# baggepinnen/LPVSpectral.jl

Measured on AMD Instinct MI355X. Metric: signals/sec, ls_sparse_spectral_lpv group lasso N=2^20 Nf=512 Nv=8 (2000 ADMM iters; iters/sec in admm_iters_per_sec), higher is better.
Workload: dtype f64

## Files before the change

lpvspectral.jl_amd/csrc/admm.hip:

```cpp
#include "lpvs_internal.h"
#include "admm_device.h"
#include "admm_host.h"

#include <algorithm>
#include <map>
#include <mutex>
#include <tuple>
#include <vector>
#include <cmath>
#include <cstdlib>
#include <string>
#include <type_traits>

namespace lpvs {

namespace {

template <int RPW>
__global__ void __launch_bounds__(256)
symv_kernel(const double *__restrict__ M, int64_t np, const double *__restrict__ rhs_all, double *__restrict__ x_all,
            const AdmmStatus *status) {
    const int sg = blockIdx.y;
    if (status != nullptr && status[sg].converged) return;
    const double *rhs = rhs_all + (int64_t)sg * np;
// ... 1536 lines not shown
void launch_symv_raw(const double *M, int64_t np, const double *rhs, double *x, const AdmmStatus *st, int ns,
                            hipStream_t s) {
    if (np >= 4096)
        hipLaunchKernelGGL(symv_kernel<4>, dim3((unsigned)ceil_div(np, 16), (unsigned)ns), dim3(256), 0, s, M, np, rhs, x, st);
    else
        hipLaunchKernelGGL(symv_kernel<1>, dim3((unsigned)ceil_div(np, 4), (unsigned)ns), dim3(256), 0, s, M, np, rhs, x, st);
}

int32_t launch_symv(const double *M, int64_t np, const double *rhs, double *x, hipStream_t s, int ns) {
    launch_symv_raw(M, np, rhs, x, nullptr, ns, s);
    LPVS_HIP(hipGetLastError());
    return LPVS_OK;
}
__global__ void __launch_bounds__(256)
rhs_from_state_kernel(const double *__restrict__ z, const double *__restrict__ u, double mu, int64_t n, int64_t np, double *__restrict__ rhs) {
    const int64_t i = (int64_t)blockIdx.x * 256 + threadIdx.x;
    if (i < np) rhs[i] = i < n ? (z[i] - u[i]) / mu : 0.0;
}
__global__ void __launch_bounds__(256)
vec_diff_kernel(const double *a, const double *b, double *out, int64_t total) {
    const int64_t i = (int64_t)blockIdx.x * 256 + threadIdx.x;
    if (i < total) out[i] = a[i] - b[i];
}
int32_t launch_nibble_refresh(const AdmmParams &p, bool from_state, const double *u_src, hipStream_t s, bool split) {
    if (p.ns != 1 || p.mp_types == nullptr || p.xb_corr == nullptr || p.nib_rhs == nullptr || p.nib_part == nullptr) { set_error("nibble refresh: not a single-signal mixed-storage handle"); return LPVS_ESTATE; }
    const int nblk = (int)(p.np / TS);
    const unsigned ntiles = (unsigned)(nblk * (nblk + 1) / 2);
    double *part1 = p.nib_part, *part2 = part1 + (size_t)ntiles * TS;
    const double *rhs = p.rhs;
    if (from_state) {
        hipLaunchKernelGGL(rhs_from_state_kernel, dim3((unsigned)ceil_div(p.np, 256)), dim3(256), 0, s, p.z, u_src, p.mu, p.n, p.np, p.nib_rhs);
        rhs = p.nib_rhs;
    }
    launch_split(reinterpret_cast<const unsigned char *>(p.Mp), p.mp_types, rhs, p.np, ntiles, part1, part2, nullptr, s, 2);
    if (split) {
        hipLaunchKernelGGL(symv_reduce_kernel, dim3((unsigned)nblk, 1u), dim3(256), 0, s, part1, part2, nblk, (int)ntiles, p.np, p.nib_rhs, nullptr, (const double *)nullptr, 0);
        hipLaunchKernelGGL(vec_diff_kernel, dim3((unsigned)ceil_div(p.np, 256)), dim3(256), 0, s, p.xb, (const double *)p.nib_rhs, const_cast<double *>(p.xb_corr), p.np);
    } else
        hipLaunchKernelGGL(symv_reduce_kernel, dim3((unsigned)nblk, 1u), dim3(256), 0, s, part1, part2, nblk, (int)ntiles, p.np, const_cast<double *>(p.xb), nullptr, p.xb_corr, 0);
    LPVS_HIP(hipGetLastError());
    return LPVS_OK;
}

void launch_gather_tile_partials(const double *part1, const double *part2, int nblk, unsigned ntiles, int64_t np, double *out, hipStream_t s) {
    hipLaunchKernelGGL(symv_reduce_kernel, dim3((unsigned)nblk, 1u), dim3(256), 0, s, part1, part2, nblk, (int)ntiles, np, out, (const AdmmStatus *)nullptr, (const double *)nullptr, 0);
}
// ... 58 lines not shown
```

lpvspectral.jl_amd/csrc/admm_one_launch.hip:

```cpp
#include "lpvs_internal.h"
#include "admm_device.h"
#include "admm_host.h"

#include <algorithm>
#include <map>
#include <mutex>
#include <tuple>
#include <vector>
#include <cmath>
#include <cstdlib>
#include <string>
#include <type_traits>

namespace lpvs {

enum { FI_FIRST = 0, FI_MID = 1, FI_LAST = 2 };
typedef void (*FiKernel)(AdmmParams, const unsigned char *, const unsigned char *, int, int, long long, int, int, int, size_t, int);
static FiKernel fi_kernel(int mode, bool small, bool batch, bool nt, bool pa, bool f32);

__device__ __forceinline__ double wave_max(double v) {
#pragma unroll
    for (int o = 32; o > 0; o >>= 1) v = fmax(v, __shfl_xor(v, o, 64));
    return v;
}
// ... 180 lines not shown
        bnv[k] = MODE != FI_FIRST ? f.bn[pg * nbt + boff + b] : 0.0;
        recv[k] = MODE != FI_LAST ? f.rec[pg * nbt + boff + b] : make_double2(0.0, 0.0);
    }
    const double Rrow = BATCH ? f.consts[2 * sg] : p.fi_R, xbmax = BATCH ? f.consts[2 * sg + 1] : p.fi_xbmax;
    __builtin_amdgcn_sched_barrier(0);
    FixRaw fr;
    float4 fha[8], fhb[8];
    double diag_pre = 0.0;
    if (MODE != FI_LAST && F32) {
        typedef unsigned int u32x4b __attribute__((ext_vector_type(4)));
        const __amdgpu_buffer_rsrc_t rs = __builtin_amdgcn_make_buffer_rsrc(const_cast<unsigned char *>(tile), 0, TS * TS * 4, 0x00020000);
        const int off_head = ((wave * 32 + (lane >> 4)) * TS + 4 * (lane & 15)) * 4;
#pragma unroll
        for (int rg = 0; rg < 8; ++rg) {
            fha[rg] = __builtin_bit_cast(float4, (u32x4b)__builtin_amdgcn_raw_buffer_load_b128(rs, off_head, rg * (4 * TS * 4), 0));
            fhb[rg] = __builtin_bit_cast(float4, (u32x4b)__builtin_amdgcn_raw_buffer_load_b128(rs, off_head, rg * (4 * TS * 4) + 256, 0));
        }
    }
    if (MODE != FI_LAST && !F32) {
        typedef unsigned int u32x4b __attribute__((ext_vector_type(4)));
        constexpr int aux = NT ? 2 : 0;
        const int tbytes = I != J ? (int)kMixedFixedTileBytes : (prefetch_all ? (int)kMixedFixedTileBytes + TS * 8 : 0);
        const __amdgpu_buffer_rsrc_t rs = __builtin_amdgcn_make_buffer_rsrc(const_cast<unsigned char *>(tile), 0, tbytes, 0x00020000);
        const __amdgpu_buffer_rsrc_t rs_nq = __builtin_amdgcn_make_buffer_rsrc(const_cast<unsigned char *>(tile), 0, p.mp_fix32 ? 0 : tbytes, 0x00020000);
        const int gq_ = lane >> 4, c_ = lane & 15;
        const int off_head = ((wave * 32 + gq_) * TS + 4 * c_) * 4;
        const int off_nq = (int)kFixHeadBytes + (wave * 64 + lane) * 32, off_st = (int)(kFixHeadBytes + kFixNibBytes) + (wave * 4 + gq_) * 32;
        fr.nq[0] = __builtin_bit_cast(uint4, (u32x4b)__builtin_amdgcn_raw_buffer_load_b128(rs_nq, off_nq, 0, aux));
        fr.nq[1] = __builtin_bit_cast(uint4, (u32x4b)__builtin_amdgcn_raw_buffer_load_b128(rs_nq, off_nq, 16, aux));
        fr.st[0] = __builtin_bit_cast(float4, (u32x4b)__builtin_amdgcn_raw_buffer_load_b128(rs, off_st, 0, aux));
        fr.st[1] = __builtin_bit_cast(float4, (u32x4b)__builtin_amdgcn_raw_buffer_load_b128(rs, off_st, 16, aux));
#pragma unroll
        for (int rg = 0; rg < 8; ++rg) {
            fr.ha[rg] = __builtin_bit_cast(int4, (u32x4b)__builtin_amdgcn_raw_buffer_load_b128(rs, off_head, rg * (4 * TS * 4), aux));
            fr.hb[rg] = __builtin_bit_cast(int4, (u32x4b)__builtin_amdgcn_raw_buffer_load_b128(rs, off_head, rg * (4 * TS * 4) + 256, aux));
        }
        if (PA) {
            const int rgo = ((c_ & 8) ? 4 : 0) + ((c_ & 4) ? 2 : 0) + ((c_ & 2) ? 1 : 0);
            typedef unsigned int u32x2b __attribute__((ext_vector_type(2)));
            const u32x2b dw = __builtin_amdgcn_raw_buffer_load_b64(rs, (int)(kFixHeadBytes + kFixNibBytes) + TS * 4 + (wave * 32 + 4 * rgo + gq_) * 8, 0, 0);
            diag_pre = __builtin_bit_cast(double, dw);
        }
    }
    __builtin_amdgcn_sched_barrier(0);
    double mR = 0, mU = 0;
#pragma unroll
    for (int k = 0; k < NK; ++k) { mR = fmax(mR, recv[k].x); mU = fmax(mU, recv[k].y); }
// ... 53 lines not shown
            if (threadIdx.x == 0) {
                f.bn[pg1 * nbt + boff + I] = red[0][0] + red[0][1];
                f.rec[pg1 * nbt + boff + I] = make_double2(fmax(red[1][0], red[1][1]), fmax(red[2][0], red[2][1]));
            }
        }
    }
    if (MODE == FI_LAST) return;
    LPVS_TL_STAMP(2);
    if (I == J && threadIdx.x < TS) f.acc((aslot + 1) % 3)[voff + e] = 0;
    if (threadIdx.x < TS) sI[i] = rhs_v; else sJ[i] = rhs_v;
    mR = wave_max_nonneg(mR); mU = wave_max_nonneg(mU);
    double B = Rrow * ((xbmax + Rrow * mR + mU) / p.mu) * 1.000001;
    const bool bound_ok = B < 0x1p1000;
    if (!(B > 0x1p-900)) B = 0x1p-900;
    int eb = 0;
    (void)frexp(bound_ok ? B : 1.0, &eb);
    const double quantum = bound_ok ? ldexp(1.0, eb - 62) : __longlong_as_double(0x7ff8000000000000ll), invq = bound_ok ? ldexp(1.0, 62 - eb) : 0.0;
    if (blockIdx.x == 0 && threadIdx.x == 0) f.qbuf[pg * nprob + sg] = quantum;
    __syncthreads();
    LPVS_TL_STAMP(3);
    const int c = lane & 15, gq = lane >> 4;
    double rj[8], tc[8], v[8];
    const double *diag = nullptr;
    if (F32) {
#pragma unroll
        for (int k = 0; k < 4; ++k) { rj[k] = sJ[4 * c + k]; rj[4 + k] = sJ[64 + 4 * c + k]; }
#pragma unroll
        for (int k = 0; k < 8; ++k) tc[k] = 0.0;
#pragma unroll
        for (int rg = 0; rg < 8; ++rg) {
            const double ri = sI[wave * 32 + 4 * rg + gq];
            const float hh[8] = {fha[rg].x, fha[rg].y, fha[rg].z, fha[rg].w, fhb[rg].x, fhb[rg].y, fhb[rg].z, fhb[rg].w};
            double a0 = 0.0, a1 = 0.0;
#pragma unroll
            for (int k = 0; k < 8; k += 2) {
                const double m0 = (double)hh[k], m1 = (double)hh[k + 1];
                tc[k] = opaque(fma(m0, ri, tc[k]));
                tc[k + 1] = opaque(fma(m1, ri, tc[k + 1]));
                a0 = fma(m0, rj[k], a0);
                a1 = fma(m1, rj[k + 1], a1);
            }
            v[rg] = a0 + a1;
            __builtin_amdgcn_sched_barrier(0);
        }
    } else if (PA || ttype != 0) {
        if (!PA && I == J) {
            FixRaw fd;
            fix_load(tile, wave, lane, fd, p.mp_fix32 != 0 ? 1 : 0);
            fi_fixed_product(fd, sI, sJ, wave, lane, v, tc);
        } else fi_fixed_product(fr, sI, sJ, wave, lane, v, tc);
        if (ttype == 2 && !prefetch_all) diag = reinterpret_cast<const double *>(tile + kFixHeadBytes + kFixNibBytes + TS * 4);
    } else {
#pragma unroll
        for (int k = 0; k < 4; ++k) { rj[k] = sJ[4 * c + k]; rj[4 + k] = sJ[64 + 4 * c + k]; }
#pragma unroll
        for (int k = 0; k < 8; ++k) tc[k] = 0.0;
        const float *head = reinterpret_cast<const float *>(tile) + (wave * 32 + gq) * TS + 4 * c;
        const unsigned short *tail = reinterpret_cast<const unsigned short *>(tile + (size_t)TS * TS * 4) + (wave * 32 + gq) * TS + 8 * c;
#pragma unroll
        for (int half = 0; half < 2; ++half) {
            float4 ha[4], hb[4];
            uint4 lq[4];
#pragma unroll
            for (int r4 = 0; r4 < 4; ++r4) {
                const int rg = 4 * half + r4;
                ha[r4] = load16<NT, float4>(head + rg * 4 * TS);
                hb[r4] = load16<NT, float4>(head + rg * 4 * TS + 64);
                lq[r4] = load16<NT, uint4>(tail + rg * 4 * TS);
            }
// ... 37 lines not shown
    }
    if (I != J) {
#pragma unroll
        for (int m = 32, cnt = 4; m >= 16; m >>= 1, cnt >>= 1) {
            const bool up = (lane & m) != 0;
#pragma unroll
            for (int k = 0; k < cnt; ++k) {
                const double lo_ = opaque(tc[k]), hi_ = opaque(tc[k + cnt]);
                tc[k] = (up ? hi_ : lo_) + __shfl_xor(up ? lo_ : hi_, m, 64);
            }
        }
        const int col = ((lane & 32) ? 64 : 0) + 4 * c + ((lane & 16) ? 2 : 0);
        sT[wave][col] = tc[0]; sT[wave][col + 1] = tc[1];
        __syncthreads();
        if (threadIdx.x < TS) {
            const double r2 = ((sT[0][threadIdx.x] + sT[1][threadIdx.x]) + sT[2][threadIdx.x]) + sT[3][threadIdx.x];
            atomicAdd(acc_cur + voff + (int64_t)J * TS + threadIdx.x, (unsigned long long)__double2ll_rn(r2 * invq));
        }
    }
    if constexpr (NIBR && !F32) {
        if (ttype != 0) {
            __syncthreads();
            FixRaw fb;
            fix_load(tile, wave, lane, fb, 2);
            double vn[8], tn[8];
            fi_fixed_product(fb, sI, sJ, wave, lane, vn, tn);
            unsigned long long *acc_n = reinterpret_cast<unsigned long long *>(p.nib_acc);
#pragma unroll
            for (int m = 8, cnt = 4; m >= 2; m >>= 1, cnt >>= 1) {
                const bool up = (c & m) != 0;
#pragma unroll
                for (int k = 0; k < cnt; ++k) {
                    const double lo_ = opaque(vn[k]), hi_ = opaque(vn[k + cnt]);
                    vn[k] = (up ? hi_ : lo_) + __shfl_xor(up ? lo_ : hi_, m, 64);
                }
            }
            vn[0] += __shfl_xor(vn[0], 1, 64);
            if ((c & 1) == 0) {
                const int rg = ((c & 8) ? 4 : 0) + ((c & 4) ? 2 : 0) + ((c & 2) ? 1 : 0);
                atomicAdd(acc_n + voff + (int64_t)I * TS + wave * 32 + 4 * rg + gq, (unsigned long long)__double2ll_rn(vn[0] * invq));
            }
            if (I != J) {
#pragma unroll
                for (int m = 32, cnt = 4; m >= 16; m >>= 1, cnt >>= 1) {
                    const bool up = (lane & m) != 0;
#pragma unroll
                    for (int k = 0; k < cnt; ++k) {
// ... 150 lines not shown
```

lpvspectral.jl_amd/csrc/api.hip:

```cpp
#include <cmath>
#include <cstdarg>
#include <cstdio>
#include <cstdlib>
#include <cstring>
#include <ctime>
#include <map>
#include <mutex>
#include <array>
#include <thread>
#include <string>
#include <vector>

#include "lpvs_internal.h"

namespace lpvs {

static thread_local char g_err[512] = "";

void set_error(const char *fmt, ...) {
    va_list ap;
    va_start(ap, fmt);
    vsnprintf(g_err, sizeof(g_err), fmt, ap);
    va_end(ap);
}
// ... 425 lines not shown
                 h->rhs.as<double>(), h->mu, h->tol, h->prox_kind, h->prox_param, h->group_len, h->status.as<AdmmStatus>(),
                 h->scratch.as<double>(), h->part.as<double>(), sym ? h->Mp.as<double>() : nullptr, (int)h->ns};
    p.mp_f32 = sym && h->Mp_mode == kMpF32 ? 1 : 0;
    p.mp_split = sym && (h->Mp_mode == kMpSplit || h->Mp_mode == kMpMixed) ? 1 : 0;
    p.mp_types = sym && h->Mp_mode == kMpMixed ? h->Mp.as<unsigned char>() + 6 * symv_packed_doubles(h->np) : nullptr;
    p.mp_fix32 = p.mp_types != nullptr && (h->Mp_fix_bits <= 32 || h->nib_period > 0) ? 1 : 0;
    p.nib_period = p.mp_types != nullptr ? h->nib_period : 0; p.nib_ramp = h->nib_ramp; p.xb_corr = h->xb_corr.as<double>(); p.nib_rhs = h->nib_rhs.as<double>(); p.nib_part = h->nib_part.as<double>(); p.nib_acc = h->nib_acc.as<long long>();
    p.xb = sym && h->offset_form ? h->xb.as<double>() : nullptr;
    p.fi = sym && h->offset_form && h->ns == 1 && (h->Mp_mode == kMpMixed || h->Mp_mode == kMpF32) && h->fi.p ? h->fi.as<double>() : nullptr;
    p.fi_R = h->fi_R; p.fi_xbmax = h->fi_xbmax;
    p.fi_prefetch_all = sym && h->Mp_mode == kMpMixed && h->Mp_fixed_tiles == (int64_t)(symv_packed_doubles(h->np) / (128 * 128)) ? 1 : 0;
    p.opt_iteration = h->opt[LPVS_OPT_ITERATION]; p.opt_nt_loads = h->opt[LPVS_OPT_NT_LOADS];
    p.sm_ctl = !sym && h->sm_ctl.p ? h->sm_ctl.as<int>() : nullptr;
    return p;
}

int32_t factorize(lpvs_problem *h, double shift) {
    if (h->M_valid && h->M_shift == shift) return LPVS_OK;
    const int64_t np = h->np, n = h->n;
    h->Mp_valid = false; h->Mp_rowsum = 0;
    if (!h->M.p) LPVS_TRY(h->M.alloc(sizeof(double) * (size_t)np * (size_t)np));
    if (!h->work.p) LPVS_TRY(h->work.alloc(spd_inverse_work_bytes(np)));
    LPVS_HIP(hipEventRecord(h->ev[3].a, h->stream));
    LPVS_HIP(hipMemcpyAsync(h->M.p, h->G.p, sizeof(double) * (size_t)np * (size_t)np, hipMemcpyDeviceToDevice, h->stream));
    LPVS_TRY(launch_add_diag(h->M.as<double>(), np, n, shift, h->stream));
    LPVS_TRY(spd_inverse_inplace(h->M.as<double>(), np, h->work.as<double>(), h->istat.as<int>(), h->stream, &h->res->aux));
    LPVS_HIP(hipEventRecord(h->ev[3].b, h->stream));
    int st = 0;
    LPVS_HIP(hipMemcpyAsync(&st, h->istat.p, sizeof(int), hipMemcpyDeviceToHost, h->stream));
    LPVS_HIP(hipStreamSynchronize(h->stream));
    h->t_factor += h->ev[3].ms();
    if (st != 0) {
        h->M_valid = false;
        set_error("(G + %.3g I) is not positive definite (non-positive pivot in the block sweep)", shift);
        return LPVS_ENUMERIC;
    }
    h->M_valid = true; h->M_shift = shift;
    return LPVS_OK;
}

}

template <class Fill>
static int32_t create_panel_problem(lpvs_problem *h, const double *y, const double *W, int64_t N, Fill fill) {
    hipStream_t s = h->stream;
    h->np = round_up(h->n, 128);
    const GramPlan pl = make_gram_plan(h->n, N);
    const int64_t Npad = pl.ksplit * pl.rows_per_chunk;
// ... 235 lines not shown
        LPVS_TRY(copy_to_device(hi.p, sl.om_hi.data(), sizeof(double) * (size_t)sl.nsl, s));
        LPVS_TRY(copy_to_device(lo.p, sl.om_lo.data(), sizeof(double) * (size_t)sl.nsl, s));
        LPVS_TRY(copy_to_device(rhi.p, sl.omr_hi.data(), sizeof(double) * (size_t)sl.nf8, s));
        LPVS_TRY(copy_to_device(rlo.p, sl.omr_lo.data(), sizeof(double) * (size_t)sl.nf8, s));
        LPVS_TRY(copy_to_device(eps.p, sl.eps.data(), sizeof(double) * sl.eps.size(), s));
        return LPVS_OK;
    }
};

static int32_t create_lpv_impl(const double *y, int64_t ns, const double *X, const double *V, int64_t N, const double *w, int64_t Nf,
                               int64_t Nv, int32_t normalize, int32_t coulomb, int32_t device, lpvs_problem **out,
                               const double *ranges = nullptr) {
    if (N <= 0 || Nf <= 0 || Nv <= 0 || ns <= 0) { set_error("N, Nf, Nv and the number of signals must be positive"); return LPVS_EARGUMENT; }
    lpvs_problem *h = nullptr;
    LPVS_TRY(problem_begin(device, out, &h));
    struct Guard { lpvs_problem *h; ~Guard() { delete h; } } guard{h};
    hipStream_t s = h->stream;
    const int64_t nb = coulomb ? 2 * Nv : Nv;
    h->kind = 1; h->N = N; h->Nf = Nf; h->nb = nb; h->n = 2 * Nf * nb; h->np = round_up(h->n, 128); h->ns = ns;
    DevArg dy, dX, dV, dw;
    LPVS_TRY(dy.set(y, N * ns, s)); LPVS_TRY(dX.set(X, N, s)); LPVS_TRY(dV.set(V, N, s)); LPVS_TRY(dw.set(w, Nf, s));
    LPVS_TRY(h->G.alloc(sizeof(double) * (size_t)h->np * (size_t)h->np));
    LPVS_TRY(h->b.alloc(sizeof(double) * (size_t)h->np * (size_t)ns));
    LPVS_HIP(hipMemsetAsync(h->G.p, 0, h->G.bytes, s));
    LPVS_HIP(hipMemsetAsync(h->b.p, 0, h->b.bytes, s));
    LPVS_TRY(alloc_state(h));

    const int form_opt = option_in_effect(LPVS_OPT_GRAM_FORM, h->opt[LPVS_OPT_GRAM_FORM]);
    const std::string form = form_opt == LPVS_GRAM_AP ? "ap" : form_opt == LPVS_GRAM_KRS ? "krs" : form_opt == LPVS_GRAM_KR ? "kr" : "auto";
    bool use_ap = false;
    ApSlots sl;
    double xam = 0;
    if (form == "auto" || form == "ap") {
        std::vector<double> hw;
        LPVS_TRY(fetch_host(hw, w, Nf));
        double xlo, xhi;
        if (ranges) xam = ranges[3];
        else LPVS_TRY(device_minmax(dX.p, N, &xlo, &xhi, &xam, s));
        sl = make_ap_slots(hw, xam);
        use_ap = sl.ok;
        if (form == "ap" && !use_ap) { set_error("LPVS_GRAM_FORM=ap but w is not an arithmetic progression (max|eps|*max|x| = %.3g)", sl.emax * xam); return LPVS_EARGUMENT; }
    }
    if (use_ap) {
        const int64_t nf8 = sl.nf8, nsl = sl.nsl, P = nb * (nb + 1) / 2;
        const ApStep &step = sl.step;
        double lo, hi, am, gamma; std::vector<double> vc;
        DevBuf K, KK, dvc, part, tab, tabb, nwork, epsr;
        ApSlotsDev sd;
        DrainOnExit drain(s);
        LPVS_HIP(hipEventRecord(h->ev[0].a, s));
        if (ranges) { lo = ranges[0]; hi = ranges[1]; am = ranges[2]; }
        else LPVS_TRY(device_minmax(dV.p, N, &lo, &hi, &am, s));
        basis_centers(lo, hi, am, Nv, coulomb, vc, &gamma);
        const int64_t ldk = nb + 1;
        LPVS_TRY(dvc.alloc(sizeof(double) * vc.size()));
        LPVS_TRY(copy_to_device(dvc.p, vc.data(), sizeof(double) * vc.size(), s));
        LPVS_TRY(K.alloc(sizeof(double) * (size_t)N * (size_t)ldk));
        LPVS_TRY(KK.alloc(sizeof(double) * (size_t)N * (size_t)P));
        LPVS_TRY(launch_basis_table(dV.p, N, dvc.as<double>(), nb, gamma, normalize, coulomb, K.as<double>(), ldk, s));
        LPVS_TRY(launch_pair_table(K.as<double>(), ldk, nb, N, KK.as<double>(), s));
        LPVS_TRY(sd.upload(sl, s));
        LPVS_HIP(hipEventRecord(h->ev[0].b, s));
        LPVS_TRY(part.alloc(std::max(nudft_partial_bytes(N, nsl, P), nudft_partial_bytes(N, nf8, nb))));
        LPVS_TRY(tab.alloc(sizeof(double) * (size_t)nsl * (size_t)P * 4));
        LPVS_TRY(tabb.alloc(sizeof(double) * (size_t)nf8 * (size_t)nb * 4));
        LPVS_HIP(hipEventRecord(h->ev[1].a, s));
        const bool nufft_on = option_in_effect(LPVS_OPT_SLOT_SUMS, h->opt[LPVS_OPT_SLOT_SUMS]) != LPVS_SLOTS_DIRECT;
        bool nufft = nufft_on && sl.merged && nufft_applicable(N, nsl, P);
        const int nfg = nufft_grid_size(nsl);
        const double xam_ = xam;
        if (nufft) {
            LPVS_TRY(nwork.alloc(nufft_work_bytes(N, nsl, P)));
// ... 27 lines not shown
                if (rc == kNufftNonFinite) by_nufft = false;
                else if (rc != LPVS_OK) return rc;
            }
            if (!by_nufft)
                LPVS_TRY(launch_nudft(dX.p, dy.p + q * N, N, K.as<double>(), ldk, (int)nb, sd.rhi.as<double>(), sd.rlo.as<double>(), (int)nf8, step, part.as<double>(), tabb.as<double>(), s));
            LPVS_TRY(launch_ap_rhs(tabb.as<double>(), by_nufft ? epsr.as<double>() : sd.eps.as<double>(), Nf, nb, h->b.as<double>() + q * h->np, s));
        }
        LPVS_HIP(hipEventRecord(h->ev[2].b, s));
        LPVS_HIP(hipStreamSynchronize(s));
        h->t_basis = h->ev[0].ms(); h->t_gram = h->ev[1].ms(); h->t_reduce = h->ev[2].ms();
        h->gram_launches = 8.0 * (double)N * (double)nsl * (double)P;
        h->gram_flops = (double)N * (double)h->n * (double)(h->n + 1);
        guard.h = nullptr;
        *out = h;
        return LPVS_OK;
    }

    const bool krs = form != "kr" && gram_krs_fits(nb);
    const GramPlan pl = krs ? make_gram_plan_pairs(Nf, nb, N) : make_gram_plan(h->n, N);
    const int64_t Npad = pl.ksplit * pl.rows_per_chunk;

    DevBuf T, K, KK, G3, slab, scr; int64_t ldk;
    DrainOnExit drain(s);
    LPVS_HIP(hipEventRecord(h->ev[0].a, s));
    LPVS_TRY(build_lpv_tables(dX.p, dV.p, N, Npad, dw.p, Nf, Nv, normalize, coulomb, T, K, &ldk, s, ranges));
    if (krs) {
        LPVS_TRY(KK.alloc(sizeof(double) * (size_t)Npad * (size_t)pl.pairs));
        LPVS_TRY(launch_pair_table(K.as<double>(), ldk, nb, Npad, KK.as<double>(), s));
    }
    LPVS_HIP(hipEventRecord(h->ev[0].b, s));
    LPVS_TRY(slab.alloc(pl.slab_bytes));
    LPVS_TRY(scr.alloc(rhs_scratch_bytes(N, h->n)));
    if (krs) LPVS_TRY(G3.alloc(sizeof(double) * (size_t)pl.np2 * (size_t)(pl.np2 * pl.pairs)));
    struct Side { hipStream_t s = nullptr; hipEvent_t ready = nullptr, done = nullptr;
                  ~Side() { if (s) { (void)hipStreamSynchronize(s); (void)hipStreamDestroy(s); } if (ready) (void)hipEventDestroy(ready); if (done) (void)hipEventDestroy(done); } } side;
    LPVS_HIP(hipStreamCreateWithFlags(&side.s, hipStreamNonBlocking));
    LPVS_HIP(hipEventCreateWithFlags(&side.ready, hipEventDisableTiming));
    LPVS_HIP(hipEventCreateWithFlags(&side.done, hipEventDisableTiming));
    LPVS_HIP(hipEventRecord(side.ready, s));
    LPVS_HIP(hipStreamWaitEvent(side.s, side.ready, 0));
    LPVS_HIP(hipEventRecord(h->ev[1].a, s));
    if (krs) LPVS_TRY(launch_gram_krs(pl, T.as<double2>(), Nf, KK.as<double>(), nb, slab.as<double>(), s));
    else LPVS_TRY(launch_gram_kr(pl, T.as<double2>(), Nf, K.as<double>(), ldk, nb, slab.as<double>(), s));
    LPVS_HIP(hipEventRecord(h->ev[1].b, s));
    for (int64_t q = 0; q < ns; ++q)
        LPVS_TRY(launch_rhs_kr(T.as<double2>(), Nf, K.as<double>(), ldk, nb, dy.p + q * N, N, h->b.as<double>() + q * h->np, scr.as<double>(), scr.bytes, side.s));
// ... 303 lines not shown
            LPVS_HIP(hipStreamSynchronize(s));
            if (want_R) memcpy(&h->Mp_rowsum, &rbits, sizeof(double));
            size_t ndiag = 0;
            for (unsigned char t : ht) { h->Mp_fixed_tiles += t != 0; ndiag += t == 2; }
            h->Mp_fixed_diag = (int64_t)ndiag;
            h->Mp_stream_bytes = (double)h->Mp_fixed_tiles * (double)kMixedFixedTileBytes + (double)ndiag * 1024.0 +
                                 (double)(ntiles - (size_t)h->Mp_fixed_tiles) * (double)kMixedFloatTileBytes;
            const size_t nblk_ = (size_t)(h->np / 128);
            if (getenv("LPVS_TRACE")) fprintf(stderr, "[lpvs] mixed packing: %lld of %zu tiles fixed point (%zu diagonal), ns = %lld\n", (long long)h->Mp_fixed_tiles, ntiles, nblk_, (long long)h->ns);
            if (2 * (size_t)h->Mp_fixed_tiles < ntiles) {
                LPVS_TRY(launch_pack_tiles_split(h->M.as<double>(), h->np, h->Mp.as<unsigned char>(), s));
                h->Mp_fixed_tiles = 0; h->Mp_fixed_diag = 0;
                h->Mp_stream_bytes = 6.0 * (double)symv_packed_doubles(h->np);
                h->Mp_valid = true; h->Mp_mode = kMpSplit; h->Mp_demoted = true; just_demoted = true;
            }
        } else LPVS_TRY(launch_pack_tiles(h->M.as<double>(), h->np, h->Mp.as<double>(), s));
        if (!just_demoted) { h->Mp_valid = true; h->Mp_mode = mode; }
    }
    LPVS_HIP(hipMemsetAsync(h->part.p, 0, h->part.bytes, s));
    h->mu = mu; h->tol = tol; h->sign = linear_sign;
    const size_t v = sizeof(double) * (size_t)h->np * (size_t)h->ns;
    LPVS_HIP(hipMemsetAsync(h->x.p, 0, v, s));
    if (x0) LPVS_TRY(copy_state_in(h, h->x.p, x0));
    std::vector<double> hb((size_t)h->np * (size_t)h->ns, 0.0);
    LPVS_HIP(hipMemcpyAsync(hb.data(), h->b.p, v, hipMemcpyDeviceToHost, s));
    LPVS_HIP(hipStreamSynchronize(s));
    if (linear_sign < 0) for (auto &q : hb) q = -q;
    LPVS_TRY(copy_to_device(h->bs.p, hb.data(), v, s));
    h->offset_form = h->np >= kSymmetricMinNp;
    if (h->offset_form) {
        if (!h->xb.p) LPVS_TRY(h->xb.alloc(v));
        int steps = 1;
        if (const char *e = experiment_env("LPVS_XB_REFINE")) steps = atoi(e) < 0 ? 0 : atoi(e);
        h->xb_refined = steps > 0;
        LPVS_TRY(launch_offset_vector_refined(h->G.as<double>(), h->M.as<double>(), h->np, h->n, (int)h->ns, h->bs.as<double>(), h->M_shift, steps,
                                              h->xb.as<double>(), h->rhs.as<double>(), h->scratch.as<double>(), s));
        if (h->xcorr()) {
            if (!h->xb0.p) LPVS_TRY(h->xb0.alloc(v));
            if (!h->corr.p) LPVS_TRY(h->corr.alloc(3 * v));
            LPVS_HIP(hipMemcpyAsync(h->xb0.p, h->xb.p, v, hipMemcpyDeviceToDevice, s));
        }
        if (h->nib_period > 0 && h->Mp_mode == kMpMixed) {
            if (!h->xb_corr.p) LPVS_TRY(h->xb_corr.alloc(v));
            if (!h->nib_rhs.p) LPVS_TRY(h->nib_rhs.alloc(v));
            if (!h->nib_acc.p) LPVS_TRY(h->nib_acc.alloc(v));
            LPVS_HIP(hipMemsetAsync(h->nib_acc.p, 0, v, s));
            { const size_t nb = (size_t)(h->np / 128), nt = nb * (nb + 1) / 2; if (!h->nib_part.p) LPVS_TRY(h->nib_part.alloc(sizeof(double) * 2 * nt * 128)); }
            LPVS_HIP(hipMemcpyAsync(h->xb_corr.p, h->xb.p, v, hipMemcpyDeviceToDevice, s));
        } else h->nib_period = 0;
    } else { h->xcorr_base = 0; h->xcorr_every = 0; }
    h->k_enq = 0;
    if (h->offset_form && h->ns == 1 && (h->Mp_mode == kMpMixed || h->Mp_mode == kMpF32) && !h->fi.p) LPVS_TRY(h->fi.alloc(sizeof(double) * fi_doubles(h->np)));
    const AdmmParams p = make_params(h);
    LPVS_TRY(launch_admm_init(p, s));
    h->fi_sync = -1;
    if (p.fi) {
        if (h->Mp_rowsum > 0 && h->Mp_mode == kMpMixed) {
            AdmmParams pr = p; pr.fi_R = h->Mp_rowsum;
            LPVS_TRY(launch_fi_setup(pr, 0, true, s, h->Mp_rowsum));
        } else LPVS_TRY(launch_fi_setup(p, 0, true, s));
        double hc[2] = {0, 0};
        LPVS_TRY(fi_read_consts(p, hc, s));
        h->fi_R = hc[0]; h->fi_xbmax = hc[1] * (1.0 + 0x1p-20); h->fi_sync = 0;
    }
    LPVS_HIP(hipStreamSynchronize(s));
    h->inited = true;
    return LPVS_OK;
}

int32_t lpvs_admm_set_state_f64(lpvs_problem *h, const double *x, const double *z, const double *u, int64_t iters_done) {
    if (!h || !x || !z || !u) { set_error("NULL argument"); return LPVS_EARGUMENT; }
    if (!h->inited) { set_error("lpvs_admm_set_state before lpvs_admm_init"); return LPVS_ESTATE; }
    if (iters_done < 0) { set_error("iters_done must be >= 0"); return LPVS_EARGUMENT; }
    LPVS_HIP(hipSetDevice(h->device));
    hipStream_t s = h->stream;
    LPVS_TRY(copy_state_in(h, h->x.p, x));
    LPVS_TRY(copy_state_in(h, h->z.p, z));
    LPVS_TRY(copy_state_in(h, h->u.p, u));
    const AdmmParams p = make_params(h);
    LPVS_TRY(launch_admm_restate(p, iters_done, s));
    h->fi_sync = -1;
    h->k_enq = iters_done;
    if (h->xcorr() && iters_done == 0) {
        const size_t v = sizeof(double) * (size_t)h->np * (size_t)h->ns;
        LPVS_HIP(hipMemcpyAsync(h->xb.p, h->xb0.p, v, hipMemcpyDeviceToDevice, s));
        if (h->nib_period > 0 && h->xb_corr.p) {
            LPVS_HIP(hipMemcpyAsync(h->xb_corr.p, h->xb0.p, v, hipMemcpyDeviceToDevice, s));
            LPVS_HIP(hipMemsetAsync(h->nib_acc.p, 0, v, s));
// ... 1176 lines not shown
```

lpvspectral.jl_amd/csrc/linalg.hip:

```cpp
#include "lpvs_internal.h"

#include <cstdlib>
#include <map>
#include <mutex>
#include <string>
#include <vector>

namespace lpvs {

namespace {

typedef double f64x4 __attribute__((ext_vector_type(4)));
constexpr int NB = 64;

__global__ void __launch_bounds__(256)
diag_inverse_kernel(const double *__restrict__ Aall, int64_t np, int k, double *__restrict__ Pall, int *status,
                    int64_t strideA, int64_t strideW) {
    __shared__ double colp[NB], rowp[NB];
    const double *A = Aall + (int64_t)blockIdx.x * strideA;
    double *P = Pall + (int64_t)blockIdx.x * strideW;
    const double *blk = A + (int64_t)k * NB * np + (int64_t)k * NB;
    const int ti = threadIdx.x >> 4, tj = threadIdx.x & 15;
    double v[4][4];
#pragma unroll
// ... 871 lines not shown
#pragma unroll
            for (int r = 0; r < 4; ++r) {
                double *sp = A + (r_lo + i * 16 + 4 * r) * np + c_lo;
#pragma unroll
                for (int j = 0; j < 2; ++j) *reinterpret_cast<double *>(reinterpret_cast<char *>(sp + j * 16) + voffb) = acc[i][j][r];
            }
        return;
    }
#pragma unroll
    for (int i = 0; i < 2; ++i)
#pragma unroll
        for (int j = 0; j < 2; ++j)
#pragma unroll
            for (int r = 0; r < 4; ++r) {
                const int64_t row = r_lo + i * 16 + lk + 4 * r, col = c_lo + j * 16 + li;
                if (col <= row) A[row * np + col] = acc[i][j][r];
            }
}

__global__ void __launch_bounds__(256) add_diag_kernel(double *__restrict__ Mall, int64_t np, int64_t n, double shift) {
    const int64_t i = (int64_t)blockIdx.x * 256 + threadIdx.x;
    double *M = Mall + (int64_t)blockIdx.y * np * np;
    if (i < np) M[i * np + i] = i < n ? M[i * np + i] + shift : 1.0;
}

__global__ void __launch_bounds__(256) negate_mirror_kernel(double *__restrict__ Aall, int64_t np) {
    __shared__ double tile[32][33];
    double *A = Aall + (int64_t)blockIdx.z * np * np;
    const int bi = blockIdx.y, bj = blockIdx.x;
    if (bj > bi) return;
    const int tx = threadIdx.x & 31, ty = threadIdx.x >> 5;
    const int64_t r0 = (int64_t)bi * 32, c0 = (int64_t)bj * 32;
    for (int r = ty; r < 32; r += 8) {
        const double v = -A[(r0 + r) * np + c0 + tx];
        tile[r][tx] = v;
        if (bi != bj || tx <= r) A[(r0 + r) * np + c0 + tx] = v;
    }
    __syncthreads();
    for (int r = ty; r < 32; r += 8)
        if (bi != bj || tx > r) A[(c0 + r) * np + r0 + tx] = tile[tx][r];
}

__global__ void __launch_bounds__(256)
symm_matmul_kernel(const double *__restrict__ A, const double *__restrict__ B, double *__restrict__ C, int64_t np) {
    const int lane = threadIdx.x & 63, wave = threadIdx.x >> 6;
    const int64_t r0 = ((int64_t)blockIdx.y * 2 + (wave >> 1)) * 64, c0 = ((int64_t)blockIdx.x * 2 + (wave & 1)) * 64;
// ... 298 lines not shown
    } else {
        sweep64(A, np, nbatch, work, status_dev, s);
        LPVS_HIP(hipGetLastError());
    }
    hipLaunchKernelGGL(negate_mirror_kernel, dim3((unsigned)(np / 32), (unsigned)(np / 32), (unsigned)nbatch), dim3(256), 0, s, A, np);
    LPVS_HIP(hipGetLastError());
    return LPVS_OK;
}

int32_t spd_inverse_inplace_batch(double *A, int64_t np, int nbatch, double *work, int *status_dev, hipStream_t s) {
    return spd_inverse_impl(A, np, nbatch, work, status_dev, s, nullptr);
}

int32_t spd_inverse_inplace(double *A, int64_t np, double *work, int *status_dev, hipStream_t s, SweepAux *aux) {
    return spd_inverse_impl(A, np, 1, work, status_dev, s, aux);
}

int32_t launch_add_diag_batch(double *M, int64_t np, int64_t n, double shift, int nbatch, hipStream_t s) {
    hipLaunchKernelGGL(add_diag_kernel, dim3((unsigned)ceil_div(np, 256), (unsigned)nbatch), dim3(256), 0, s, M, np, n, shift);
    LPVS_HIP(hipGetLastError());
    return LPVS_OK;
}

int32_t launch_add_diag(double *M, int64_t np, int64_t n, double shift, hipStream_t s) {
    hipLaunchKernelGGL(add_diag_kernel, dim3((unsigned)ceil_div(np, 256)), dim3(256), 0, s, M, np, n, shift);
    LPVS_HIP(hipGetLastError());
    return LPVS_OK;
}

int32_t launch_symm_matmul(const double *A, const double *B, double *C, int64_t np, hipStream_t s) {
    if (np % 128 != 0) return LPVS_ESTATE;
    hipLaunchKernelGGL(symm_matmul_kernel, dim3((unsigned)(np / 128), (unsigned)(np / 128)), dim3(256), 0, s, A, B, C, np);
    LPVS_HIP(hipGetLastError());
    return LPVS_OK;
}

}
```

lpvspectral.jl_amd/csrc/lpvs_internal.h:

```cpp
#pragma once
#include <hip/hip_runtime.h>
#include <exception>
#include <new>
#include <stdint.h>
#include <functional>
#include <string>
#include <vector>

#include "../../include/lpvspectral.h"

namespace lpvs {

inline const char *experiment_env(const char *name) {
#ifdef LPVS_NO_EXPERIMENTS
    (void)name;
    return nullptr;
#else
    const char *on = getenv("LPVS_EXPERIMENTS");
    return (on && on[0] == '1') ? getenv(name) : nullptr;
#endif
}

void set_error(const char *fmt, ...);
#define LPVS_HIP(call)                                                                       \
// ... 125 lines not shown
std::vector<double> nufft_window_scale(int nf, int mode0, int nslots);
int32_t launch_nufft_window_spread(const double *x, const double *W, const double *yA, const double *yB, bool hasB, const int64_t *offs_dev, int nwin,
                                   int64_t n, double D_hi, double D_lo, int nf, double *gridA, double *gridB, int64_t grid_bstride, hipStream_t s);
int32_t launch_nufft_window_modes(const double *grids, int64_t grid_bstride, int nwin, int nf, int mode0, int nslots, const double *scale_dev, double *tab,
                                  int64_t tab_bstride, hipStream_t s);
int32_t launch_ap_assemble_fourier(const double *tab, const double *eps, int64_t Nf, int64_t s0, double delta, int zf, int64_t n, double *G,
                                   int64_t ldg, int nbatch, int64_t tab_stride, int64_t g_stride, hipStream_t s);
int32_t launch_ap_rhs_fourier(const double *tab, const double *eps, int64_t Nf, int zf, double *b, int nbatch, int64_t tab_stride,
                              int64_t b_stride, hipStream_t s);
int32_t launch_ap_assemble(const double *tab, const double *eps, int64_t Nf, int64_t s0, double delta, int64_t nb, int64_t n, double *G,
                           int64_t ldg, hipStream_t s);
int32_t launch_ap_rhs(const double *tab, const double *eps, int64_t Nf, int64_t nb, double *b, hipStream_t s);

struct SweepAux {
    hipStream_t side = nullptr;
    hipStream_t bulk = nullptr;
    hipEvent_t panel = nullptr, rest = nullptr, band = nullptr, second = nullptr, bulkdone = nullptr;
    int32_t ensure();
    ~SweepAux();
};
size_t spd_inverse_work_bytes(int64_t np);
int32_t spd_inverse_inplace(double *A, int64_t np, double *work, int *status_dev, hipStream_t s, SweepAux *aux = nullptr);
int32_t launch_add_diag(double *M, int64_t np, int64_t n, double shift, hipStream_t s);
int32_t launch_add_diag_batch(double *M, int64_t np, int64_t n, double shift, int nbatch, hipStream_t s);
int32_t spd_inverse_inplace_batch(double *A, int64_t np, int nbatch, double *work, int *status_dev, hipStream_t s);
int32_t launch_symm_matmul(const double *A, const double *B, double *C, int64_t np, hipStream_t s);

struct AdmmStatus {
    long long iters;
    int converged;
    int pad;
    double nxz;
};
struct AdmmParams {
    const double *M;
    int64_t np;
    int64_t n;
    const double *b;
    double *x, *z, *u, *rhs;
    double mu, tol;
    int prox_kind;
    double prox_param;
    int64_t group_len;
    AdmmStatus *status;
    double *scratch;
    double *part;
    const double *Mp;
    int ns;
    int mp_f32 = 0;
    int mp_split = 0;
    int nib_period = 0;
    int nib_ramp = 0;
    const double *xb_corr = nullptr;
    double *nib_rhs = nullptr;
    long long *nib_acc = nullptr;
    double *nib_part = nullptr;
    int mp_fix32 = 0;
    const unsigned char *mp_types = nullptr;
    const double *xb = nullptr;
    double *fi = nullptr;
    long long fi_base = 0;
    double fi_R = 0, fi_xbmax = 0;
    int fi_prefetch_all = 0;
    int opt_iteration = 0, opt_nt_loads = 0;
    int *sm_ctl = nullptr;
};
bool small_iter_applicable(const AdmmParams &p);
int32_t launch_nibble_refresh(const AdmmParams &p, bool from_state, const double *u_src, hipStream_t s, bool split = false);
inline bool nib_refresh_due(long long g, int period, int ramp) {
    if (period <= 0) return false;
    if (ramp <= 0) return g == 1 || g % period == 0;
    long long p2 = 1;
    while (2 * p2 <= g) p2 *= 2;
    long long step = p2 / ramp;
    if (step < 1) step = 1;
    if (step > period) step = period;
    return g % step == 0;
}
bool nib_fused_applies(const AdmmParams &p);
int32_t launch_xupdate_correction(const AdmmParams &p, const double *G, double shift, const double *b, const double *xb0, double *xb_eff, double *t, hipStream_t s);
size_t fi_doubles(int64_t np, int64_t nprob = 1);
bool fi_applicable(const AdmmParams &p);
int32_t launch_fi_setup(const AdmmParams &p, long long base, bool with_consts, hipStream_t s, double r_known = -1.0);
int32_t fi_read_consts(const AdmmParams &p, double out[2], hipStream_t s);
size_t symv_part_doubles(int64_t np, int64_t ns = 1);
size_t symv_packed_doubles(int64_t np);
int32_t launch_pack_tiles(const double *M, int64_t np, double *Mp, hipStream_t s);
int32_t launch_pack_tiles_f32(const double *M, int64_t np, float *Mp, hipStream_t s);
int32_t launch_pack_tiles_split(const double *M, int64_t np, unsigned char *Mp, hipStream_t s);
int32_t launch_pack_tiles_mixed(const double *M, int64_t np, unsigned char *Mp, unsigned char *types, unsigned long long *absmax, hipStream_t s,
                                bool diag_float = false, double *abs_part = nullptr, int64_t n_valid = 0, double *rows_scratch = nullptr, int fix_bits = 36);
// ... 81 lines not shown
```

Baseline: 14.33.

## Trim setup copies, memsets and host round-trips; reuse nibble tile loads

Setup now copies G into M in one fused kernel that adds the diagonal shift and touches only the lower-triangle tiles, replacing a full device-to-device copy plus a separate diagonal kernel. The sign flip of b runs on the device instead of going through a host round-trip. The full G memset becomes a memset of only the padding rows and columns on the Fourier path, and a redundant stream sync is dropped. In the fused iteration kernel, the nibble-refresh path reuses nibble and scale registers loaded earlier instead of reloading the tile. The lower-only copy assumes nothing reads M's upper triangle before the inverse, and it requires np to be a multiple of 128.

```diff
diff --git a/lpvspectral.jl_amd/csrc/admm.hip b/lpvspectral.jl_amd/csrc/admm.hip
--- a/lpvspectral.jl_amd/csrc/admm.hip
+++ b/lpvspectral.jl_amd/csrc/admm.hip
@@ -1582,6 +1582,16 @@
     const int64_t i = (int64_t)blockIdx.x * 256 + threadIdx.x;
     if (i < total) out[i] = a[i] - b[i];
 }
+__global__ void __launch_bounds__(256)
+signed_copy_kernel(const double *__restrict__ in, int negate, double *__restrict__ out, int64_t total) {
+    const int64_t i = (int64_t)blockIdx.x * 256 + threadIdx.x;
+    if (i < total) out[i] = negate ? -in[i] : in[i];
+}
+int32_t launch_signed_copy(const double *in, int sign, double *out, int64_t total, hipStream_t s) {
+    hipLaunchKernelGGL(signed_copy_kernel, dim3((unsigned)ceil_div(total, 256)), dim3(256), 0, s, in, sign < 0 ? 1 : 0, out, total);
+    LPVS_HIP(hipGetLastError());
+    return LPVS_OK;
+}
 int32_t launch_nibble_refresh(const AdmmParams &p, bool from_state, const double *u_src, hipStream_t s, bool split) {
     if (p.ns != 1 || p.mp_types == nullptr || p.xb_corr == nullptr || p.nib_rhs == nullptr || p.nib_part == nullptr) { set_error("nibble refresh: not a single-signal mixed-storage handle"); return LPVS_ESTATE; }
     const int nblk = (int)(p.np / TS);
diff --git a/lpvspectral.jl_amd/csrc/admm_one_launch.hip b/lpvspectral.jl_amd/csrc/admm_one_launch.hip
--- a/lpvspectral.jl_amd/csrc/admm_one_launch.hip
+++ b/lpvspectral.jl_amd/csrc/admm_one_launch.hip
@@ -226,7 +226,7 @@
         constexpr int aux = NT ? 2 : 0;
         const int tbytes = I != J ? (int)kMixedFixedTileBytes : (prefetch_all ? (int)kMixedFixedTileBytes + TS * 8 : 0);
         const __amdgpu_buffer_rsrc_t rs = __builtin_amdgcn_make_buffer_rsrc(const_cast<unsigned char *>(tile), 0, tbytes, 0x00020000);
-        const __amdgpu_buffer_rsrc_t rs_nq = __builtin_amdgcn_make_buffer_rsrc(const_cast<unsigned char *>(tile), 0, p.mp_fix32 ? 0 : tbytes, 0x00020000);
+        const __amdgpu_buffer_rsrc_t rs_nq = __builtin_amdgcn_make_buffer_rsrc(const_cast<unsigned char *>(tile), 0, (!NIBR && p.mp_fix32) ? 0 : tbytes, 0x00020000);
         const int gq_ = lane >> 4, c_ = lane & 15;
         const int off_head = ((wave * 32 + gq_) * TS + 4 * c_) * 4;
         const int off_nq = (int)kFixHeadBytes + (wave * 64 + lane) * 32, off_st = (int)(kFixHeadBytes + kFixNibBytes) + (wave * 4 + gq_) * 32;
@@ -326,6 +326,8 @@
     const int c = lane & 15, gq = lane >> 4;
     double rj[8], tc[8], v[8];
     const double *diag = nullptr;
+    uint4 nib_nq[2] = {make_uint4(0, 0, 0, 0), make_uint4(0, 0, 0, 0)};
+    float4 nib_st[2] = {make_float4(0, 0, 0, 0), make_float4(0, 0, 0, 0)};
     if (F32) {
 #pragma unroll
         for (int k = 0; k < 4; ++k) { rj[k] = sJ[4 * c + k]; rj[4 + k] = sJ[64 + 4 * c + k]; }
@@ -348,7 +350,22 @@
             __builtin_amdgcn_sched_barrier(0);
         }
     } else if (PA || ttype != 0) {
-        if (!PA && I == J) {
+        if constexpr (NIBR) {
+            const bool z32 = p.mp_fix32 != 0;
+            const uint4 zero4 = make_uint4(0, 0, 0, 0);
+            if (!PA && I == J) {
+                FixRaw fd;
+                fix_load(tile, wave, lane, fd, 0);
+                nib_nq[0] = fd.nq[0]; nib_nq[1] = fd.nq[1]; nib_st[0] = fd.st[0]; nib_st[1] = fd.st[1];
+                if (z32) { fd.nq[0] = zero4; fd.nq[1] = zero4; }
+                fi_fixed_product(fd, sI, sJ, wave, lane, v, tc);
+            } else {
+                nib_nq[0] = fr.nq[0]; nib_nq[1] = fr.nq[1]; nib_st[0] = fr.st[0]; nib_st[1] = fr.st[1];
+                FixRaw f0 = fr;
+                if (z32) { f0.nq[0] = zero4; f0.nq[1] = zero4; }
+                fi_fixed_product(f0, sI, sJ, wave, lane, v, tc);
+            }
+        } else if (!PA && I == J) {
             FixRaw fd;
             fix_load(tile, wave, lane, fd, p.mp_fix32 != 0 ? 1 : 0);
             fi_fixed_product(fd, sI, sJ, wave, lane, v, tc);
@@ -432,7 +449,10 @@
         if (ttype != 0) {
             __syncthreads();
             FixRaw fb;
-            fix_load(tile, wave, lane, fb, 2);
+            fb.nq[0] = nib_nq[0]; fb.nq[1] = nib_nq[1]; fb.st[0] = nib_st[0]; fb.st[1] = nib_st[1];
+            const int bias = (int)0x80000000u;
+#pragma unroll
+            for (int rg = 0; rg < 8; ++rg) { fb.ha[rg] = make_int4(bias, bias, bias, bias); fb.hb[rg] = fb.ha[rg]; }
             double vn[8], tn[8];
             fi_fixed_product(fb, sI, sJ, wave, lane, vn, tn);
             unsigned long long *acc_n = reinterpret_cast<unsigned long long *>(p.nib_acc);
diff --git a/lpvspectral.jl_amd/csrc/api.hip b/lpvspectral.jl_amd/csrc/api.hip
--- a/lpvspectral.jl_amd/csrc/api.hip
+++ b/lpvspectral.jl_amd/csrc/api.hip
@@ -471,8 +471,7 @@
     if (!h->M.p) LPVS_TRY(h->M.alloc(sizeof(double) * (size_t)np * (size_t)np));
     if (!h->work.p) LPVS_TRY(h->work.alloc(spd_inverse_work_bytes(np)));
     LPVS_HIP(hipEventRecord(h->ev[3].a, h->stream));
-    LPVS_HIP(hipMemcpyAsync(h->M.p, h->G.p, sizeof(double) * (size_t)np * (size_t)np, hipMemcpyDeviceToDevice, h->stream));
-    LPVS_TRY(launch_add_diag(h->M.as<double>(), np, n, shift, h->stream));
+    LPVS_TRY(launch_shifted_lower_copy(h->G.as<double>(), h->M.as<double>(), np, n, shift, h->stream));
     LPVS_TRY(spd_inverse_inplace(h->M.as<double>(), np, h->work.as<double>(), h->istat.as<int>(), h->stream, &h->res->aux));
     LPVS_HIP(hipEventRecord(h->ev[3].b, h->stream));
     int st = 0;
@@ -754,7 +753,6 @@
     LPVS_TRY(dy.set(y, N * ns, s)); LPVS_TRY(dX.set(X, N, s)); LPVS_TRY(dV.set(V, N, s)); LPVS_TRY(dw.set(w, Nf, s));
     LPVS_TRY(h->G.alloc(sizeof(double) * (size_t)h->np * (size_t)h->np));
     LPVS_TRY(h->b.alloc(sizeof(double) * (size_t)h->np * (size_t)ns));
-    LPVS_HIP(hipMemsetAsync(h->G.p, 0, h->G.bytes, s));
     LPVS_HIP(hipMemsetAsync(h->b.p, 0, h->b.bytes, s));
     LPVS_TRY(alloc_state(h));
 
@@ -780,6 +778,11 @@
         DevBuf K, KK, dvc, part, tab, tabb, nwork, epsr;
         ApSlotsDev sd;
         DrainOnExit drain(s);
+        if (h->np > h->n) {
+            const size_t npz = (size_t)h->np, nz = (size_t)h->n;
+            LPVS_HIP(hipMemsetAsync(h->G.as<double>() + nz * npz, 0, sizeof(double) * (npz - nz) * npz, s));
+            LPVS_HIP(hipMemset2DAsync(h->G.as<double>() + nz, sizeof(double) * npz, 0, sizeof(double) * (npz - nz), nz, s));
+        }
         LPVS_HIP(hipEventRecord(h->ev[0].a, s));
         if (ranges) { lo = ranges[0]; hi = ranges[1]; am = ranges[2]; }
         else LPVS_TRY(device_minmax(dV.p, N, &lo, &hi, &am, s));
@@ -853,6 +856,7 @@
 
     DevBuf T, K, KK, G3, slab, scr; int64_t ldk;
     DrainOnExit drain(s);
+    LPVS_HIP(hipMemsetAsync(h->G.p, 0, h->G.bytes, s));
     LPVS_HIP(hipEventRecord(h->ev[0].a, s));
     LPVS_TRY(build_lpv_tables(dX.p, dV.p, N, Npad, dw.p, Nf, Nv, normalize, coulomb, T, K, &ldk, s, ranges));
     if (krs) {
@@ -1202,11 +1206,7 @@
     const size_t v = sizeof(double) * (size_t)h->np * (size_t)h->ns;
     LPVS_HIP(hipMemsetAsync(h->x.p, 0, v, s));
     if (x0) LPVS_TRY(copy_state_in(h, h->x.p, x0));
-    std::vector<double> hb((size_t)h->np * (size_t)h->ns, 0.0);
-    LPVS_HIP(hipMemcpyAsync(hb.data(), h->b.p, v, hipMemcpyDeviceToHost, s));
-    LPVS_HIP(hipStreamSynchronize(s));
-    if (linear_sign < 0) for (auto &q : hb) q = -q;
-    LPVS_TRY(copy_to_device(h->bs.p, hb.data(), v, s));
+    LPVS_TRY(launch_signed_copy(h->b.as<double>(), linear_sign, h->bs.as<double>(), h->np * h->ns, s));
     h->offset_form = h->np >= kSymmetricMinNp;
     if (h->offset_form) {
         if (!h->xb.p) LPVS_TRY(h->xb.alloc(v));
@@ -1242,8 +1242,7 @@
         double hc[2] = {0, 0};
         LPVS_TRY(fi_read_consts(p, hc, s));
         h->fi_R = hc[0]; h->fi_xbmax = hc[1] * (1.0 + 0x1p-20); h->fi_sync = 0;
-    }
-    LPVS_HIP(hipStreamSynchronize(s));
+    } else LPVS_HIP(hipStreamSynchronize(s));
     h->inited = true;
     return LPVS_OK;
 }
diff --git a/lpvspectral.jl_amd/csrc/linalg.hip b/lpvspectral.jl_amd/csrc/linalg.hip
--- a/lpvspectral.jl_amd/csrc/linalg.hip
+++ b/lpvspectral.jl_amd/csrc/linalg.hip
@@ -917,6 +917,22 @@
     const int64_t i = (int64_t)blockIdx.x * 256 + threadIdx.x;
     double *M = Mall + (int64_t)blockIdx.y * np * np;
     if (i < np) M[i * np + i] = i < n ? M[i * np + i] + shift : 1.0;
+}
+
+__global__ void __launch_bounds__(256)
+shifted_lower_copy_kernel(const double *__restrict__ G, double *__restrict__ M, int64_t np, int64_t n, double shift) {
+    const int64_t c0 = (int64_t)blockIdx.x * 256, r0 = (int64_t)blockIdx.y * 16;
+    if (c0 > (r0 / 256) * 256) return;
+    const int64_t c = c0 + 2 * (threadIdx.x & 127);
+    if (c >= np) return;
+#pragma unroll
+    for (int k = 0; k < 8; ++k) {
+        const int64_t r = r0 + 2 * k + (threadIdx.x >> 7);
+        double2 v = *reinterpret_cast<const double2 *>(G + r * np + c);
+        if (r == c) v.x = r < n ? v.x + shift : 1.0;
+        if (r == c + 1) v.y = r < n ? v.y + shift : 1.0;
+        *reinterpret_cast<double2 *>(M + r * np + c) = v;
+    }
 }
 
 __global__ void __launch_bounds__(256) negate_mirror_kernel(double *__restrict__ Aall, int64_t np) {
@@ -1261,6 +1277,13 @@
     return LPVS_OK;
 }
 
+int32_t launch_shifted_lower_copy(const double *G, double *M, int64_t np, int64_t n, double shift, hipStream_t s) {
+    if (np % 128 != 0) { set_error("shifted_lower_copy: np=%lld not a multiple of 128", (long long)np); return LPVS_ESTATE; }
+    hipLaunchKernelGGL(shifted_lower_copy_kernel, dim3((unsigned)ceil_div(np, 256), (unsigned)(np / 16)), dim3(256), 0, s, G, M, np, n, shift);
+    LPVS_HIP(hipGetLastError());
+    return LPVS_OK;
+}
+
 int32_t launch_add_diag(double *M, int64_t np, int64_t n, double shift, hipStream_t s) {
     hipLaunchKernelGGL(add_diag_kernel, dim3((unsigned)ceil_div(np, 256)), dim3(256), 0, s, M, np, n, shift);
     LPVS_HIP(hipGetLastError());
diff --git a/lpvspectral.jl_amd/csrc/lpvs_internal.h b/lpvspectral.jl_amd/csrc/lpvs_internal.h
--- a/lpvspectral.jl_amd/csrc/lpvs_internal.h
+++ b/lpvspectral.jl_amd/csrc/lpvs_internal.h
@@ -171,6 +171,7 @@
 size_t spd_inverse_work_bytes(int64_t np);
 int32_t spd_inverse_inplace(double *A, int64_t np, double *work, int *status_dev, hipStream_t s, SweepAux *aux = nullptr);
 int32_t launch_add_diag(double *M, int64_t np, int64_t n, double shift, hipStream_t s);
+int32_t launch_shifted_lower_copy(const double *G, double *M, int64_t np, int64_t n, double shift, hipStream_t s);
 int32_t launch_add_diag_batch(double *M, int64_t np, int64_t n, double shift, int nbatch, hipStream_t s);
 int32_t spd_inverse_inplace_batch(double *A, int64_t np, int nbatch, double *work, int *status_dev, hipStream_t s);
 int32_t launch_symm_matmul(const double *A, const double *B, double *C, int64_t np, hipStream_t s);
@@ -216,6 +217,7 @@
 };
 bool small_iter_applicable(const AdmmParams &p);
 int32_t launch_nibble_refresh(const AdmmParams &p, bool from_state, const double *u_src, hipStream_t s, bool split = false);
+int32_t launch_signed_copy(const double *in, int sign, double *out, int64_t total, hipStream_t s);
 inline bool nib_refresh_due(long long g, int period, int ramp) {
     if (period <= 0) return false;
     if (ramp <= 0) return g == 1 || g % period == 0;
```

Result: no change. 14.41 (median of 6 runs) (+0.5%).
